# DerrickWang005/CRIS.pytorch

Hardware: AMD Instinct MI355X
Metric: train-step samples/sec, CRIS-R50 416x416 bs=64; loss parity vs ref (higher is better)
Workload: dtype bf16; 1 GPU; CRIS-R50 bf16 training step (fwd+BCE+bwd+Adam), 416x416, per-GPU bs=8, 17-token text, synthetic RefCOCO-shape batch resident in HBM (BASELINE.json configs[1]); global_batch=8, parallelism=dp1, launch=graph, graph_captured=True, syncbn_exchange=none, grad_exchange=none

## Files before the change

cris/pytorch_amd/csrc/build.py:

```python
import hashlib
import os
import subprocess
import sys

HERE = os.path.dirname(os.path.abspath(__file__))
SOURCES = ["api.hip", "gemm.hip", "gemm8.hip", "gemm_fp8.hip", "wgrad.hip", "norm.hip", "attention.hip", "elementwise.hip", "ema.hip", "lr.hip", "smallf32.hip", "evalpost.hip", "inputpipe.hip", "p2p.hip", "comm.hip", "jpeg.hip", "png.hip"]
LIB = os.path.join(HERE, "libcris_hip.so")
STAMP = os.path.join(HERE, ".build_stamp")
FLAGS = ["--offload-arch=gfx950", "-O3", "-std=c++17", "-fPIC", "-Wno-unused-result", "-fno-slp-vectorize", "-fno-vectorize"]
FLAGS += os.environ.get("CRIS_EXTRA_HIPCC_FLAGS", "").split()
OBJDUMP = "/opt/rocm/lib/llvm/bin/llvm-objdump"


def _digest():
    h = hashlib.sha256()
    for f in SOURCES + ["common.h", "gemm_common.h", "p2p_ll.h", "jpeg_core.h", os.path.join("..", "..", "..", "include", "cris_hip.h")]:
        with open(os.path.join(HERE, f), "rb") as fh:
            h.update(fh.read())
    h.update(" ".join(FLAGS).encode())
    return h.hexdigest()


def _current(dig):
    return os.path.exists(LIB) and os.path.exists(STAMP) and open(STAMP).read() == dig


def build(force=False, verbose=False):
    dig = _digest()
    if not force and _current(dig):
        return LIB
    import fcntl
    with open(os.path.join(HERE, ".build_lock"), "w") as lock:
        fcntl.flock(lock, fcntl.LOCK_EX)
        try:
            if not force and _current(dig):
                return LIB
            return _compile(dig, verbose)
        finally:
            fcntl.flock(lock, fcntl.LOCK_UN)


def packed_fp32_ops(lib=LIB):
    import re
    import shutil
    import tempfile
    if not os.path.exists(OBJDUMP):
        return None
    found = {}
    with tempfile.TemporaryDirectory() as td:
        so = os.path.join(td, "lib.so")
        shutil.copy(lib, so)
        subprocess.run([OBJDUMP, "--offloading", so], cwd=td, stdout=subprocess.DEVNULL, stderr=subprocess.DEVNULL)
        for f in sorted(os.listdir(td)):
            if "gfx950" not in f:
                continue
            asm = subprocess.run([OBJDUMP, "-d", os.path.join(td, f)], stdout=subprocess.PIPE, stderr=subprocess.DEVNULL).stdout.decode()
            name = "?"
            for line in asm.splitlines():
                m = re.match(r"^[0-9a-f]+ <(.*)>:", line)
# ... 49 lines not shown
```

cris/pytorch_amd/csrc/gemm.hip:

```cpp
#include "gemm_common.h"
#ifndef ST_64x64
#define ST_64x64 3
#endif
#ifndef ST_64x128
#define ST_64x128 3
#endif
#ifndef ST_128x64
#define ST_128x64 3
#endif
#ifndef ST_128x128
#define ST_128x128 2
#endif
#define SKINNY_MAX_M 144

#ifdef G4_PROBE
__device__ unsigned long long* g4_stamps;
#define G4_T(k) t_stamp[k] = __builtin_amdgcn_s_memtime()
#ifndef G4_ABL
#define G4_ABL 0
#endif
#else
#define G4_T(k)
#define G4_ABL 0
#endif


template <int BM, int BN, int WAVES_M, int WAVES_N, int STAGES, int EPI, int MT_ = 32, int KS = 1>
__device__ __forceinline__ void conv_gemm_tile(const cris_conv_gemm_params& p, int bid, unsigned char* smem) {
    constexpr int WTM = BM / WAVES_M;
    constexpr int WTN = BN / WAVES_N;
    constexpr int MT = MT_;
    using acc_t = typename std::conditional<MT == 32, f32x16, f32x4>::type;
    constexpr int FM = WTM / MT;
    constexpr int FN = WTN / MT;
    constexpr int NA = BM / 32;
    constexpr int NB = BN / 32;
    constexpr int A_BYTES = BM * 128;
    constexpr int STAGE_BYTES = (BM + BN) * 128;

#ifdef G4_PROBE
    unsigned long long t_stamp[6];
#endif
    G4_T(0);
    if (G4_ABL & 8) {
        if (p.M < 0) p.colsum[0] = 0.f;
        return;
    }
    const int t = threadIdx.x;
    const int lane = t & 63;
    const int wave = (t >> 6) & 3;
    const int grp = KS > 1 ? (t >> 8) : 0;
    unsigned char* const ring = smem + grp * (STAGES * STAGE_BYTES);
    const int wm = wave / WAVES_N;
    const int wn = wave % WAVES_N;

    const int tiles_n = (p.N + BN - 1) / BN;
    const int tiles_m = (p.M + BM - 1) / BM;
    int tile_m, tile_n;
    if ((long)p.N * p.K > (1L << 20)) {
        tile_n = cris_fast_div(bid, tiles_m, __builtin_amdgcn_rcpf((float)tiles_m));
        tile_m = bid - tile_n * tiles_m;
    } else {
        tile_m = cris_fast_div(bid, tiles_n, __builtin_amdgcn_rcpf((float)tiles_n));
        tile_n = bid - tile_m * tiles_n;
// ... 370 lines not shown
    }
    __syncthreads();
    if (wave == 0) {
        float* slab = p.ws + ((size_t)ks * gridDim.x + nb) * (FM * FN * 256);
#pragma unroll
        for (int i = 0; i < FM; ++i)
#pragma unroll
            for (int j = 0; j < FN; ++j) {
                f32x4 v = acc[i][j];
#pragma unroll
                for (int w = 0; w < SK2_WAVES - 1; ++w) {
                    const f32x4 o = *reinterpret_cast<const f32x4*>(&red[w][i * FN + j][lane][0]);
                    v[0] += o[0]; v[1] += o[1]; v[2] += o[2]; v[3] += o[3];
                }
                *reinterpret_cast<f32x4*>(slab + (i * FN + j) * 256 + lane * 4) = v;
            }
    }
}

template <int FM>
__global__ __launch_bounds__(256) void skinny_finish_kernel(const cris_conv_gemm_params p, int nslices, int nblocks) {
    const int lane = threadIdx.x & 63, wave = threadIdx.x >> 6;
    const int u = blockIdx.x * 4 + wave;
    const int nfc = nblocks * 2;
    if (u >= FM * nfc) return;
    const int i = u / nfc, c = u - i * nfc;
    const int nb = c >> 1, j = c & 1;
    f32x4 one[1][1];
    one[0][0] = (f32x4){0.f, 0.f, 0.f, 0.f};
    const float* src = p.ws + (size_t)nb * (FM * 2 * 256) + (i * 2 + j) * 256 + lane * 4;
    const size_t slab = (size_t)nblocks * (FM * 2 * 256);
    for (int k0 = 0; k0 < nslices; k0 += 4) {
        f32x4 o[4];
#pragma unroll
        for (int q = 0; q < 4; ++q) o[q] = *reinterpret_cast<const f32x4*>(src + (size_t)min(k0 + q, nslices - 1) * slab);
#pragma unroll
        for (int q = 0; q < 4; ++q)
            if (k0 + q < nslices) { one[0][0][0] += o[q][0]; one[0][0][1] += o[q][1]; one[0][0][2] += o[q][2]; one[0][0][3] += o[q][3]; }
    }
    gemm_epilogue<0, 16, 1, 1>(p, one, i * 16, c * 16, i, lane);
}

static int skinny_split_slices(const cris_conv_gemm_params& p) {
    static const int target = cris_env_int("CRIS_SKINNY_BLOCKS", 192);
    const int nblocks = cris_cdiv(p.N, 32);
    int ks = target / nblocks;
    const int kmax = p.K / 128;
    if (ks > kmax) ks = kmax;
    if (ks < 1) ks = 1;
    return ks;
}
static int skinny_kslice(const cris_conv_gemm_params& p, int slices) { return cris_cdiv(cris_cdiv(p.K, slices), 32) * 32; }

enum { V_SKINNY1 = 0, V_SKINNY9, V_SKINNY9S, V_128x64, V_64x64, V_64x128, V_128x128, V_8W_256x256, V_8W_256x128, V_8W_128x256, V_8W_128x128, V_64x64_K2, V_COUNT };

#define CRIS_TILE4_KERNS(K, BM, BN, WM, WN, ST) K<BM, BN, WM, WN, ST, 0>, K<BM, BN, WM, WN, ST, 1>, K<BM, BN, WM, WN, ST, 2>
#define CRIS_TILE4_ROW(NAME, BM, BN, WM, WN, ST)                                                                           \
    {NAME, BM, BN, 256, ST * (BM + BN) * 128, BM / WM, 8,                                                                  \
     {CRIS_TILE4_KERNS(conv_gemm_kernel, BM, BN, WM, WN, ST), conv_gemm_kernel<BM, BN, WM, WN, ST, 3>},                  \
     {CRIS_TILE4_KERNS(conv_gemm_group_kernel, BM, BN, WM, WN, ST)}}
static const cris_gemm_variant_desc* variant_table() {
    static const cris_gemm_variant_desc* const g8 = cris_gemm8_variants();
    static const cris_gemm_variant_desc tab[V_COUNT] = {
        {"skinny1", 16, 32, 64 * SK_WAVES, 0, 16, 8, {}, {}},
        {"skinny9", SKINNY_MAX_M, 32, 64 * SK_WAVES, 0, 16, 8, {}, {}},
        {"skinny9s", SKINNY_MAX_M, 32, 64 * SK2_WAVES, 0, 16, 8, {}, {}},
        CRIS_TILE4_ROW("128x64", 128, 64, 4, 1, ST_128x64),
        CRIS_TILE4_ROW("64x64", 64, 64, 2, 2, ST_64x64),
        CRIS_TILE4_ROW("64x128", 64, 128, 2, 2, ST_64x128),
        CRIS_TILE4_ROW("128x128", 128, 128, 2, 2, ST_128x128),
        g8[0], g8[1], g8[2], g8[3],
        {"64x64k2", 64, 64, 512, 2 * 2 * (64 + 64) * 128, 32, 8,
         {conv_gemm_kernel<64, 64, 2, 2, 2, 0, 32, 2>, conv_gemm_kernel<64, 64, 2, 2, 2, 1, 32, 2>, conv_gemm_kernel<64, 64, 2, 2, 2, 2, 32, 2>, nullptr},
         {}}};
    return tab;
}
static int variants_lds_ready() {
    static const int rc = [] {
        int rc = 0;
        for (int v = 0; v < V_COUNT; ++v) {
            const cris_gemm_variant_desc& r = variant_table()[v];
            for (int e = 0; e < 4; ++e) rc |= cris_set_lds((const void*)r.kern[e], r.lds_bytes);
            for (int e = 0; e < 3; ++e) rc |= cris_set_lds((const void*)r.group_kern[e], r.lds_bytes);
        }
        return rc;
    }();
    if (rc != 0) cris_set_error("gemm variants: hipFuncSetAttribute(MaxDynamicSharedMemorySize) failed (%d)", rc);
    return rc;
}

static int epilogue_kind(const cris_conv_gemm_params& p) {
    const bool plain = p.drop_thresh == 0u && !p.outT && p.out && !p.out_f32 && !(p.resid && p.resid_f32);
    if (plain && !p.bias && p.act == 0) return p.bnr_y ? 3 : 1;
    return !plain ? 0 : (p.act == 0 || p.act == 1 || p.act == 3) ? 2 : 0;
}

static bool variant_applicable(int v, const cris_conv_gemm_params& p) {
    if (v < 0 || v >= V_COUNT) return false;
    const cris_gemm_variant_desc& r = variant_table()[v];
    if (r.kern[0]) return p.C % r.c_mult == 0;
    const bool lin = p.KH == 1 && p.KW == 1 && p.stride == 1 && p.pad == 0 && p.OH == p.H && p.OW == p.W;
    return lin && p.M <= r.bm;
}

static int pick_variant(const cris_conv_gemm_params& p) {
    const bool lin = p.KH == 1 && p.KW == 1 && p.stride == 1 && p.pad == 0 && p.OH == p.H && p.OW == p.W;
    if (lin && p.M <= 16) return V_SKINNY1;
    static const int skinny_split = cris_env_int("CRIS_SKINNY_SPLIT", 1);
    if (lin && p.M <= SKINNY_MAX_M) {
        if (!skinny_split) return V_SKINNY9;
        return p.K >= 1024 ? V_SKINNY9S : V_64x64;
    }
    static const int g8 = cris_env_int("CRIS_GEMM8", 1);
    static const int g8_min = cris_env_int("CRIS_GEMM8_MIN_TILES", 150);
    static const int g8_min_k = cris_env_int("CRIS_GEMM8_MIN_K", 256);
    static const int g8_t128_lo = cris_env_int("CRIS_GEMM8_T128_LO", 100), g8_t128_hi = cris_env_int("CRIS_GEMM8_T128_HI", 216);
    if (g8 && epilogue_kind(p) != 0 && (p.C & 63) == 0 && p.N >= 128) {
        const long t128 = (long)cris_cdiv(p.M, 128) * cris_cdiv(p.N, 128);
        if (p.K >= 512 && t128 >= g8_t128_lo && t128 <= g8_t128_hi) return V_8W_128x128;
        if (p.N > 128 && p.K >= g8_min_k) {
            const long t256 = (long)cris_cdiv(p.M, 256) * cris_cdiv(p.N, 256);
            if (p.K >= 512 && t256 >= g8_min && !(t256 > 256 && t256 <= 400)) return V_8W_256x256;
            const long t128x256 = (long)cris_cdiv(p.M, 128) * cris_cdiv(p.N, 256);
            if (t128x256 >= g8_min && !(t128x256 > 256 && t128x256 <= 400) && (p.K >= 512 || t128x256 <= 256)) return V_8W_128x256;
        }
    }
    static const int narrow128 = cris_env_int("CRIS_GEMM_NARROW_128", 0);
    if (p.N <= 64) return narrow128 ? V_128x64 : V_64x64;
    static const int t128_min = cris_env_int("CRIS_GEMM_T128_MIN", 448);
    if (p.M <= 8192 || (long)cris_cdiv(p.M, 128) * cris_cdiv(p.N, 128) < t128_min) {
        static const int t64_max = cris_env_int("CRIS_GEMM_T64_MAX", 1024);
        const bool long_k = p.K >= 4096 && p.M >= 4096 && p.N >= 256;
        if (!long_k && (long)cris_cdiv(p.M, 64) * cris_cdiv(p.N, 128) < t64_max) {
            static const int ks2 = cris_env_int("CRIS_GEMM_KS2", 0), ks2_max = cris_env_int("CRIS_GEMM_KS2_MAX_BLOCKS", 512);
            static const int ks2_min_k = cris_env_int("CRIS_GEMM_KS2_MIN_K", 256);
            if (ks2 && p.K >= ks2_min_k && epilogue_kind(p) != 3 && (long)cris_cdiv(p.M, 64) * cris_cdiv(p.N, 64) <= ks2_max) return V_64x64_K2;
            return V_64x64;
        }
        return V_64x128;
    }
    return V_128x128;
}
static int variant_stat_rows(int v) { return variant_table()[v].stat_rows; }
static int resolve_variant(const cris_conv_gemm_params& p, int variant) {
    if (variant < 0) return pick_variant(p);
    return variant_applicable(variant, p) ? variant : -1;
}
extern "C" int cris_conv_gemm_stat_rows(const cris_conv_gemm_params* p) { return variant_stat_rows(pick_variant(*p)); }
extern "C" int cris_conv_gemm_variant_stat_rows(const cris_conv_gemm_params* p, int variant) {
    const int v = resolve_variant(*p, variant);
    return v < 0 ? -1 : variant_stat_rows(v);
}
extern "C" long cris_conv_gemm_ws_floats(const cris_conv_gemm_params* p, int variant) {
    const int v = resolve_variant(*p, variant);
    if (v != V_SKINNY9S) return 0;
    return (long)skinny_split_slices(*p) * cris_cdiv(p->N, 32) * (9 * 2 * 256);
}
extern "C" int cris_conv_gemm_plan(const cris_conv_gemm_params* p, int variant, int* epilogue) {
    if (epilogue) *epilogue = epilogue_kind(*p);
    return resolve_variant(*p, variant);
}
extern "C" int cris_conv_gemm_num_variants(void) { return V_COUNT; }
extern "C" const char* cris_conv_gemm_variant_name(int v) { return (v >= 0 && v < V_COUNT) ? variant_table()[v].name : "?"; }

extern "C" int cris_conv_gemm(const cris_conv_gemm_params* pp, void* stream) { return cris_conv_gemm_variant(pp, -1, stream); }

static int conv_gemm_check(const cris_conv_gemm_params& p);

extern "C" int cris_conv_gemm_group_launch(const cris_conv_gemm_group* gp, int variant, void* stream) {
    CRIS_CHECK_ARG(gp && gp->n > 0 && gp->n <= CRIS_GEMM_GROUP_MAX, "1 .. CRIS_GEMM_GROUP_MAX problems per launch");
    CRIS_CHECK_ARG(variant >= 0 && variant < V_COUNT && variant_table()[variant].group_kern[0],
                   "group launches run the 4-wave tiles or the 8-wave 128x128 tile");
    if (gp->n == 1) return cris_conv_gemm_variant(&gp->prob[0], variant, stream);
    const cris_gemm_variant_desc& r = variant_table()[variant];
    cris_conv_gemm_group g = *gp;
    const int epi = epilogue_kind(g.prob[0]);
    CRIS_CHECK_ARG(epi < 3, "BatchNorm-backward partials are not available in grouped launches");
    int start = 0;
    for (int i = 0; i < g.n; ++i) {
        const cris_conv_gemm_params& p = g.prob[i];
        if (conv_gemm_check(p) != 0) return -1;
        CRIS_CHECK_ARG(epilogue_kind(p) == epi, "the problems of a group must share the epilogue instantiation");
        CRIS_CHECK_ARG(variant_applicable(variant, p), "tile variant not applicable to a problem of the group");
        g.block_start[i] = start;
        start += cris_tile_blocks(r.bm, r.bn, p.M, p.N);
    }
    for (int i = g.n; i <= CRIS_GEMM_GROUP_MAX; ++i) g.block_start[i] = start;
    if (const int rc = variants_lds_ready()) return rc;
    return cris_launch_tile(r.group_kern[epi], start, r.threads, r.lds_bytes, (hipStream_t)stream, g);
}

static int conv_gemm_check(const cris_conv_gemm_params& p) {
    CRIS_CHECK_ARG(p.A && p.Wt, "null operand");
    CRIS_CHECK_ARG(p.M > 0 && p.N > 0 && p.K > 0, "empty problem");
    CRIS_CHECK_ARG((p.C & 7) == 0 && (p.lda & 7) == 0 && (p.a_coff & 7) == 0, "A channels/ld/offset must be multiples of 8");
    CRIS_CHECK_ARG((p.ldb & 7) == 0 && (p.K & 7) == 0 && p.ldb >= p.K, "W ld / K must be multiples of 8");
    CRIS_CHECK_ARG(p.K == p.KH * p.KW * p.C, "K != KH*KW*C");
    CRIS_CHECK_ARG(p.M == p.Bn * p.OH * p.OW, "M != Bn*OH*OW");
    CRIS_CHECK_ARG(p.M < (1 << 24) && (long)cris_cdiv(p.M, 64) * cris_cdiv(p.N, 64) < (1L << 22),
                   "more than 2^24 output rows / 2^22 tiles (the reciprocal index arithmetic of the prologue is exact below that)");
    CRIS_CHECK_ARG(p.out || p.outT || p.colsum, "no output");
    CRIS_CHECK_ARG(!p.bnr_y || (epilogue_kind(p) == 3 && p.colsum && p.colsq && p.bnr_mean && p.bnr_invstd && p.bnr_scale && p.bnr_shift &&
                                (p.bnr_ldy & 7) == 0 && (size_t)p.M * p.bnr_ldy * 2 < (1UL << 31)),
                   "BatchNorm-backward partials need the lean epilogue, both tables and the four coefficient vectors");
    CRIS_CHECK_ARG(p.stat_ld == 0 || p.stat_ld >= p.N, "stat_ld < N");
    CRIS_CHECK_ARG(!p.outT || ((p.T_E & 63) == 0 && p.T_L > 0 && (p.T_Lpad & 3) == 0 && p.T_Lpad >= p.T_L && p.M % p.T_L == 0),
                   "bad transposed-store geometry");
    CRIS_CHECK_ARG((uintptr_t)p.A % 16 == 0 && (uintptr_t)p.Wt % 16 == 0, "operands must be 16-byte aligned");
    CRIS_CHECK_ARG((long)p.M * p.N < (1L << 32) || p.drop_thresh == 0u, "dropout index overflow");
    CRIS_CHECK_ARG((size_t)p.Bn * p.H * p.W * p.lda * 2 < (1UL << 31) && ((size_t)p.N + 256) * p.ldb * 2 < (1UL << 31) &&
                       (!p.out || (size_t)p.M * p.ldc * 4 < (1UL << 31)) && (!p.resid || (size_t)p.M * p.ldr * 4 < (1UL << 31)),
                   "operand extent must stay below 2 GiB (32-bit buffer offsets)");
    return 0;
}

extern "C" int cris_conv_gemm_variant(const cris_conv_gemm_params* pp, int variant, void* stream) {
    const cris_conv_gemm_params& p = *pp;
    if (conv_gemm_check(p) != 0) return -1;
    hipStream_t s = (hipStream_t)stream;
    if (const int rc = variants_lds_ready()) return rc;
    int v = resolve_variant(p, variant);
    CRIS_CHECK_ARG(v >= 0, "tile variant not applicable to this problem");
    if (variant < 0 && v == V_SKINNY9S && !p.ws) v = V_SKINNY9;
    const cris_gemm_variant_desc& r = variant_table()[v];
    CRIS_CHECK_ARG(!p.bnr_y || r.kern[3],
                   "BatchNorm-backward partials: the 4-wave tiles and the 8-wave 128x128 tile only (cris_conv_gemm_plan tells which variant runs)");
    const int nblocks = cris_cdiv(p.N, r.bn);
    switch (v) {
        case V_SKINNY1: return cris_launch_tile(skinny_gemm_kernel<1>, nblocks, r.threads, 0, s, p);
        case V_SKINNY9: return cris_launch_tile(skinny_gemm_kernel<9>, nblocks, r.threads, 0, s, p);
        case V_SKINNY9S: {
            CRIS_CHECK_ARG(p.ws != nullptr, "the split-K skinny variant needs the workspace (cris_conv_gemm_ws_floats)");
            const int slices = skinny_split_slices(p);
            hipLaunchKernelGGL(skinny_split_kernel<9>, dim3(nblocks, slices), dim3(r.threads), 0, s, p, skinny_kslice(p, slices));
            hipLaunchKernelGGL(skinny_finish_kernel<9>, dim3(cris_cdiv(9 * nblocks * 2, 4)), dim3(256), 0, s, p, slices, nblocks);
            CRIS_LAUNCH_CHECK();
            return 0;
        }
        default: return cris_launch_tile(r.kern[epilogue_kind(p)], cris_tile_blocks(r.bm, r.bn, p.M, p.N), r.threads, r.lds_bytes, s, p);
    }
}

#define PACK_ELEMS 4096

__global__ __launch_bounds__(256) void pack_weights_kernel(const cris_pack_desc* __restrict__ tab, int n_desc) {
    int lo = 0, hi = n_desc - 1;
    const int bid = blockIdx.x;
    while (lo < hi) {
        const int mid = (lo + hi + 1) >> 1;
        if (tab[mid].block_start <= bid) lo = mid; else hi = mid - 1;
    }
    const cris_pack_desc d = tab[lo];
    const int lb = bid - d.block_start;
    const long nF = d.dstF ? (long)d.N * d.taps * d.Cpad : 0;
    const long blocksF = (nF + PACK_ELEMS - 1) / PACK_ELEMS;
    if (lb < blocksF) {
        const long base = (long)lb * PACK_ELEMS;
        for (int e = threadIdx.x; e < PACK_ELEMS; e += 256) {
            const long i = base + e;
            if (i >= nF) break;
            const int c = (int)(i % d.Cpad);
            const long r = i / d.Cpad;
            const int tap = (int)(r % d.taps);
            const int n = (int)(r / d.taps);
            float v = 0.f;
            if (c < d.Cin) v = d.src_transposed ? d.src[(size_t)c * d.N + n] : d.src[((size_t)n * d.Cin + c) * d.taps + tap];
            if (d.row_scale) v *= d.row_scale[n];
            const long ldF = d.ldF > 0 ? d.ldF : (long)d.taps * d.Cpad;
            d.dstF[(long)n * ldF + (long)tap * d.Cpad + c] = f2bf(v);
        }
    } else {
        __shared__ float tile[64][65];
        const int tn = (d.Npad + 63) / 64, tc = (d.Cin + 63) / 64;
        int r = lb - (int)blocksF;
        const int nt = r % tn; r /= tn;
        const int ct = r % tc;
// ... 40 lines not shown
```

cris/pytorch_amd/csrc/gemm_common.h:

```cpp
#pragma once
#include "common.h"
#include "../../../include/cris_hip.h"
#include <type_traits>

#define BK 64
#ifndef CRIS_FAST_EPILOGUE
#define CRIS_FAST_EPILOGUE 1
#endif
#ifndef CRIS_FAST_EPILOGUE_GEN
#define CRIS_FAST_EPILOGUE_GEN 1
#endif

__device__ __forceinline__ int cris_xcd_logical_block(int bid, int total) {
    const int q = total >> 3, r = total & 7;
    const int xcd = bid & 7, idx = bid >> 3;
    return (xcd < r ? xcd * (q + 1) : r * (q + 1) + (xcd - r) * q) + idx;
}

__device__ __forceinline__ int lds_off(int row, int chunk) {
    return row * 128 + (((chunk ^ (row >> 1)) & 7) << 4);
}

__device__ __forceinline__ bf16_t f2bf_hw(float x) { return __builtin_bit_cast(bf16_t, (__bf16)x); }

// ... 324 lines not shown
                    b0 += gg;
                    b1 += gg * ((yv[r] - b_mean) * b_inv);
                }
            }
            if (MT == 16) { b0 += __shfl_xor(b0, 16, 64); b1 += __shfl_xor(b1, 16, 64); }
            b0 += __shfl_xor(b0, 32, 64);
            b1 += __shfl_xor(b1, 32, 64);
            if (fg == 0 && cvalid && part_cnt > 0) {
                p.colsum[(size_t)part * sld + col] = b0;
                p.colsq[(size_t)part * sld + col] = b1;
            }
        } else if (p.colsum) {
            float s1 = 0.f;
#pragma unroll
            for (int ig = 0; ig < FM * NG; ++ig)
#pragma unroll
                for (int r = 0; r < 4; ++r) s1 += vals[ig][r];
            if (MT == 16) s1 += __shfl_xor(s1, 16, 64);
            s1 += __shfl_xor(s1, 32, 64);
            const float mu = part_cnt > 0 ? s1 / (float)part_cnt : 0.f;
            float q = 0.f;
#pragma unroll
            for (int ig = 0; ig < FM * NG; ++ig)
#pragma unroll
                for (int r = 0; r < 4; ++r) {
                    const int i = ig / NG, g = ig % NG;
                    const int m = row0 + i * MT + (MT == 16 ? fg * 4 : g * 8 + fg * 4) + r;
                    const float d = vals[ig][r] - mu;
                    q += (m < p.M) ? d * d : 0.f;
                }
            if (MT == 16) q += __shfl_xor(q, 16, 64);
            q += __shfl_xor(q, 32, 64);
            if (fg == 0 && cvalid && part_cnt > 0) {
                const int sld = p.stat_ld ? p.stat_ld : p.N;
                p.colsum[(size_t)part * sld + col] = s1;
                p.colsq[(size_t)part * sld + col] = q;
            }
        }
    }
}


typedef void (*cris_gemm_kern_t)(const cris_conv_gemm_params);
typedef void (*cris_gemm_group_kern_t)(const cris_conv_gemm_group);
struct cris_gemm_variant_desc {
    const char* name;
    int bm, bn;
    int threads, lds_bytes;
    int stat_rows;
    int c_mult;
    cris_gemm_kern_t kern[4];
    cris_gemm_group_kern_t group_kern[3];
};
const cris_gemm_variant_desc* cris_gemm8_variants();

static inline int cris_tile_blocks(int bm, int bn, int M, int N) { return cris_cdiv(M, bm) * cris_cdiv(N, bn); }
static inline int cris_set_lds(const void* kern, int bytes) {
    return kern ? (int)hipFuncSetAttribute(kern, hipFuncAttributeMaxDynamicSharedMemorySize, bytes) : 0;
}
template <typename KERN, typename ARG>
static int cris_launch_tile(KERN kern, int blocks, int threads, int lds_bytes, hipStream_t s, const ARG& arg) {
    hipLaunchKernelGGL(kern, dim3(blocks), dim3(threads), lds_bytes, s, arg);
    CRIS_LAUNCH_CHECK();
    return 0;
}
```

cris/pytorch_amd/hip.py:

```python
import contextlib
import ctypes as C
import os

import torch

_HERE = os.path.dirname(os.path.abspath(__file__))
LIB_PATH = os.path.join(_HERE, "csrc", "libcris_hip.so")
if os.environ.get("CRIS_LIB_VARIANT"):
    LIB_PATH = os.path.join(_HERE, "csrc", "variants", "libcris_hip_%s.so" % os.environ["CRIS_LIB_VARIANT"])

P, I, L, F, U = C.c_void_p, C.c_int, C.c_long, C.c_float, C.c_uint32


class ConvGemmParams(C.Structure):
    _fields_ = [("A", P), ("Wt", P), ("bias", P), ("resid", P), ("out", P), ("outT", P), ("colsum", P), ("colsq", P),
                ("T_sec_stride", L),
                ("lda", I), ("a_coff", I),
                ("Bn", I), ("H", I), ("W", I), ("C", I),
                ("OH", I), ("OW", I), ("KH", I), ("KW", I), ("stride", I), ("pad", I),
                ("ldb", I),
                ("M", I), ("N", I), ("K", I),
                ("act", I),
                ("ldr", I), ("r_coff", I), ("resid_f32", I),
                ("ldc", I), ("c_coff", I), ("out_f32", I),
# ... 193 lines not shown

class JpegImage(C.Structure):
    _fields_ = [("coef", P), ("planes", P), ("rgb", P), ("info", JpegInfo)]


class P2PParams(C.Structure):
    _fields_ = [("data", P), ("boxes", P), ("gen_dev", P), ("err", P),
                ("n", I), ("rank", I), ("world", I),
                ("slot", I), ("slots", I),
                ("max_floats", I),
                ("gen_host", I),
                ("spin_limit", I)]


class P2PLink(C.Structure):
    _fields_ = [("boxes", P), ("err", P), ("gen_dev", P),
                ("gen_host", I), ("rank", I), ("world", I),
                ("slot", I), ("slots", I), ("max_floats", I), ("spin_limit", I)]


class P2PArenaParams(C.Structure):
    _fields_ = [("arenas", P), ("lo", C.c_long), ("n", C.c_long), ("link", P2PLink), ("blocks", I)]


STRUCTS = {
    "cris_conv_gemm_params": ConvGemmParams, "cris_conv_gemm_group": ConvGemmGroup, "cris_wgrad_params": WgradParams, "cris_wgrad_group": WgradGroup, "cris_pack_desc": PackDesc,
    "cris_conv_gemm_fp8_params": ConvGemmFp8Params, "cris_pack_fp8_desc": PackFp8Desc,
    "cris_bn_apply_params": BnApplyParams, "cris_bn_bwd_params": BnBwdParams, "cris_ln_fwd_params": LnFwdParams,
    "cris_ln_bwd_params": LnBwdParams, "cris_sum_entry": SumEntry, "cris_sum_group": SumGroup, "cris_attn_params": AttnParams, "cris_adam_desc": AdamDesc, "cris_ema_desc": EmaDesc, "cris_p2p_params": P2PParams, "cris_p2p_link": P2PLink, "cris_p2p_arena_params": P2PArenaParams, "cris_zero_ranges": ZeroRanges,
    "cris_sample_desc": SampleDesc, "cris_eval_desc": EvalDesc, "cris_jpeg_info": JpegInfo, "cris_jpeg_image": JpegImage,
}

_SIGS = {
    "cris_last_error": (C.c_char_p, []),
    "cris_abi_version": (I, []),
    "cris_sizeof": (I, [C.c_char_p]),
    "cris_echo_conv_gemm": (L, [P]),
    "cris_conv_gemm": (I, [P, P]),
    "cris_conv_wgrad": (I, [P, P]),
    "cris_conv_wgrad_group": (I, [P, P]),
    "cris_conv_wgrad_tile": (I, [P]),
    "cris_wgrad_reduce": (I, [P, P]),
    "cris_wgrad_reduce_group": (I, [P, P]),
    "cris_wgrad_ws_floats": (L, [I, I, I, I]),
    "cris_pack_weights": (I, [P, I, I, P]),
    "cris_pack_blocks": (I, [P]),
    "cris_pack_block_elems": (I, []),
    "cris_conv_gemm_stat_rows": (I, [P]),
    "cris_conv_gemm_variant": (I, [P, I, P]),
    "cris_conv_gemm_variant_stat_rows": (I, [P, I]),
    "cris_conv_gemm_ws_floats": (L, [P, I]),
    "cris_conv_gemm_num_variants": (I, []),
    "cris_conv_gemm_plan": (I, [P, I, P]),
    "cris_conv_gemm_group_launch": (I, [P, I, P]),
    "cris_conv_gemm_variant_name": (C.c_char_p, [I]),
    "cris_conv_gemm_fp8": (I, [P, I, P]),
    "cris_conv_gemm_fp8_plan": (I, [P, I]),
    "cris_conv_gemm_fp8_num_variants": (I, []),
    "cris_conv_gemm_fp8_variant_name": (C.c_char_p, [I]),
    "cris_pack_weights_fp8": (I, [P, I, I, P]),
    "cris_avgpool2_fwd_fp8": (I, [P, I, I, I, I, I, I, P, I, I, P, I, I, I, P]),
    "cris_absmax_bf16": (I, [P, I, I, L, I, P, P, P]),
    "cris_absmax_ws_floats": (I, []),
    "cris_bn_partials_rows": (I, [I]),
    "cris_bn_finalize": (I, [P, P, I, I, F, F, P, P, P, P, F, F, I, P, P, P, P, P, P, P]),
    "cris_bn_sync_pack": (I, [P, P, P, F, I, P]),
    "cris_bn_sync_unpack": (I, [P, P, F, I, P]),
    "cris_colstats_bf16": (I, [P, I, I, I, I, I, P, P, P]),
    "cris_bn_eval_coeffs": (I, [P, P, P, P, F, I, P, P, P]),
    "cris_bn_apply": (I, [P, P]),
    "cris_bn_bwd_reduce": (I, [P, P]),
    "cris_bn_bwd_apply": (I, [P, P]),
    "cris_bn_bwd_ws_floats": (L, [P]),
    "cris_ln_bwd_parts": (I, [I]),
    "cris_sum_tables": (I, [P, P]),
    "cris_ln_fwd": (I, [P, P]),
    "cris_ln_bwd": (I, [P, P]),
    "cris_attn_fwd": (I, [P, P]),
    "cris_attn_bwd_dq": (I, [P, P]),
    "cris_attn_bwd_dkv": (I, [P, P]),
    "cris_stem_im2col": (I, [P, I, I, I, P, P]),
    "cris_avgpool2_fwd": (I, [P, I, I, I, I, I, I, P, I, I, P]),
    "cris_avgpool2_bwd": (I, [P, I, I, I, I, I, I, P, I, I, I, P]),
    "cris_upsample2_fwd": (I, [P, I, I, I, I, I, I, P, I, I, P]),
    "cris_upsample2_bwd": (I, [P, I, I, I, I, I, I, P, I, I, I, P]),
    "cris_fill_coords": (I, [P, I, I, I, I, I, I, P]),
    "cris_gather_samples_bf16": (I, [P, I, I, P, I, I, I, P, I, I, P]),
    "cris_add_bf16": (I, [P, I, I, P, I, I, P, I, I, I, I, P]),
    "cris_add_rowtable": (I, [P, I, P, I, P, I, I, I, P]),
    "cris_cast_f32_bf16": (I, [P, P, L, P]),
    "cris_cast_bf16_f32": (I, [P, P, L, I, P]),
    "cris_cast_f32_bf16_drop": (I, [P, P, L, F, U, U, U, P, P]),
    "cris_step_advance": (I, [P, P, P, P]),
    "cris_step_advance_micro": (I, [P, P, P, I, I, P]),
    "cris_axpy_f32": (I, [P, P, F, L, P]),
    "cris_grad_accumulate": (I, [P, P, L, I, P]),
    "cris_quickgelu_fwd": (I, [P, P, L, P]),
    "cris_quickgelu_bwd": (I, [P, P, P, L, P]),
    "cris_embed_fwd": (I, [P, P, P, I, I, I, P, P]),
    "cris_embed_bwd": (I, [P, P, I, I, I, P, P, P, P]),
    "cris_eot_gather": (I, [P, P, I, I, I, P, P, P]),
    "cris_eot_scatter_add": (I, [P, P, I, I, I, P, P]),
    "cris_eot_gather_ln_f32": (I, [P, P, P, P, P, P, I, I, I, P, P, P]),
    "cris_eot_scatter_add_f32": (I, [P, P, I, I, I, P, P]),
    "cris_linear_f32_small": (I, [P, I, P, I, I, P, I, I, I, P, I, I, P]),
    "cris_outer_sum_f32_small": (I, [P, I, P, I, I, I, I, P, I, P, P]),
# ... 159 lines not shown
```

cris/pytorch_amd/ops.py:

```python
from __future__ import annotations

import ctypes as C
import math
import os
from dataclasses import dataclass
from typing import Optional

import torch

from . import hip
from .hip import ptr

BF16 = torch.bfloat16


def _stream():
    return torch.cuda.current_stream().cuda_stream


def pad8(n: int) -> int:
    return (n + 7) // 8 * 8


def pad32(n: int) -> int:
# ... 55 lines not shown
    def __init__(self):
        self.items = []

    @classmethod
    def groupable(cls):
        if cls.GROUPABLE is None:
            names = gemm_variants()
            cls.GROUPABLE = {names.index(n) for n in ("128x64", "64x64", "64x128", "128x128", "8w128x128")}
        return cls.GROUPABLE

    def add(self, p, variant, keep, flops, nbytes, tag):
        epi = C.c_int(0)
        v = hip.load().cris_conv_gemm_plan(C.byref(p), variant, C.byref(epi))
        if v < 0:
            raise ValueError("GEMM tile variant %r cannot run this problem" % (variant,))
        self.items.append((p, v, epi.value, keep, flops, nbytes, tag))

    def __len__(self):
        return len(self.items)

    def flush(self):
        items, self.items = self.items, []
        if not items:
            return
        groups = {}
        for it in items:
            key = (it[1], it[2]) if (self.enabled and it[1] in self.groupable()) else ("solo", id(it))
            groups.setdefault(key, []).append(it)
        for key, its in groups.items():
            if key[0] == "solo":
                _launch_gemm(its[0][0], its[0][1], its[0][4], its[0][5], its[0][6])
                continue
            its.sort(key=lambda it: -it[0].K)
            for i in range(0, len(its), hip.GEMM_GROUP_MAX):
                chunk = its[i:i + hip.GEMM_GROUP_MAX]
                if len(chunk) == 1:
                    _launch_gemm(chunk[0][0], chunk[0][1], chunk[0][4], chunk[0][5], chunk[0][6])
                    continue
                grp = hip.ConvGemmGroup()
                grp.n = len(chunk)
                for j, it in enumerate(chunk):
                    grp.prob[j] = it[0]
                if KERNEL_TIMER is not None:
                    KERNEL_TIMER.launch("conv_gemm", sum(it[4] for it in chunk), sum(it[5] for it in chunk), "cris_conv_gemm_group_launch",
                                        C.byref(grp), key[0], tag="group of %d: %s" % (len(chunk), " + ".join(it[6] for it in chunk)), tile=True)
                else:
                    hip.call("cris_conv_gemm_group_launch", C.byref(grp), key[0], _stream())


def _launch_gemm(p, variant, flops, nbytes, tag):
    if KERNEL_TIMER is not None:
        v = hip.load().cris_conv_gemm_plan(C.byref(p), variant, None)
        KERNEL_TIMER.launch("skinny_gemm" if (p.M <= 144 and p.KH == 1) else "conv_gemm", flops, nbytes, "cris_conv_gemm_variant",
                            C.byref(p), variant, tag=tag, tile=gemm_variants()[v] not in ("skinny1", "skinny9", "skinny9s"))
        return
    hip.call("cris_conv_gemm_variant", C.byref(p), variant, _stream())


def conv_gemm(A, Wt, g: Geom, N: int, *, lda=None, a_coff=0, ldb=None, bias=None, act=0, resid=None, ldr=None, r_coff=0,
              out=None, ldc=None, c_coff=0, outT=None, T_L=0, T_Lpad=0, T_E=0, T_sec_stride=0, stats=False,
              drop: Drop = NO_DROP, variant: int = -1, queue: Optional[GemmQueue] = None, bnr: Optional[dict] = None):
    p = hip.ConvGemmParams()
    p.A, p.Wt, p.bias = ptr(A), ptr(Wt), ptr(bias)
    p.lda = lda if lda is not None else A.shape[-1]
    p.a_coff = a_coff
    p.Bn, p.H, p.W, p.C = g.Bn, g.H, g.W, g.C
    p.OH, p.OW, p.KH, p.KW, p.stride, p.pad = g.OH, g.OW, g.KH, g.KW, g.stride, g.pad
    p.ldb = ldb if ldb is not None else Wt.shape[-1]
    p.M, p.N, p.K = g.M, N, g.K
    p.act = act
    if resid is not None:
        p.resid = ptr(resid)
        p.ldr = ldr if ldr is not None else resid.shape[-1]
        p.r_coff = r_coff
        p.resid_f32 = 1 if resid.dtype == torch.float32 else 0
    if out is not None:
        p.out = ptr(out)
        p.ldc = ldc if ldc is not None else out.shape[-1]
        p.c_coff = c_coff
        p.out_f32 = 1 if out.dtype == torch.float32 else 0
    if outT is not None:
        p.outT = ptr(outT)
        p.T_L, p.T_Lpad, p.T_E, p.T_sec_stride = T_L, T_Lpad, T_E, T_sec_stride
    p.drop_p, p.drop_thresh, p.drop_seed, p.drop_stream = drop.p, drop.thresh, drop.seed & 0xFFFFFFFF, drop.stream
    p.drop_seed_dev = ptr(drop.dev)
    st = None
    if isinstance(variant, str):
        variant = gemm_variants().index(variant)
    rows = hip.load().cris_conv_gemm_variant_stat_rows(C.byref(p), variant)
    if rows < 0:
        raise ValueError("GEMM tile variant %r cannot run this problem" % (variant,))
    parts = None
    if bnr is not None:
        assert not stats
        epi = C.c_int(0)
        v = hip.load().cris_conv_gemm_plan(C.byref(p), variant, C.byref(epi))
        nparts = (g.M + rows - 1) // rows
        if gemm_variants()[v] not in ("128x64", "64x64", "64x128", "128x128", "8w128x128") or epi.value != 1 or nparts > BNR_MAX_PARTS:
            bnr = None
        else:
            parts = BnrParts(torch.empty(nparts, 2 * N, dtype=torch.float32, device=A.device), nparts)
            p.colsum, p.colsq, p.stat_ld = ptr(parts.t), parts.t.data_ptr() + 4 * N, 2 * N
            p.bnr_y, p.bnr_ldy, p.bnr_coff = ptr(bnr["y"]), bnr["ldy"], bnr["coff"]
            p.bnr_mean, p.bnr_invstd, p.bnr_scale, p.bnr_shift = ptr(bnr["mean"]), ptr(bnr["invstd"]), ptr(bnr["scale"]), ptr(bnr["shift"])
    if stats:
        st = Stats((g.M + rows - 1) // rows, N, rows, A.device)
        p.colsum, p.colsq = ptr(st[0]), ptr(st[1])
    nws = hip.load().cris_conv_gemm_ws_floats(C.byref(p), variant)
    ws = torch.empty(nws, dtype=torch.float32, device=A.device) if nws else None
    p.ws = ptr(ws)
    flops, nbytes, tag = 2.0 * g.M * N * g.K, 2.0 * (g.M * g.C + N * g.K + g.M * N), "M%d N%d K%d k%d" % (g.M, N, g.K, g.KH)
    if queue is not None:
        assert bnr is None and parts is None, "a queued launch cannot feed a BatchNorm backward that runs before the flush"
        queue.add(p, variant, (A, Wt, bias, resid, out, outT, drop.dev, ws, st.t if st is not None else None), flops, nbytes, tag)
        return st
    _launch_gemm(p, variant, flops, nbytes, tag)
    return parts if bnr is not None else st


BNR_MAX_PARTS = int(os.environ.get("CRIS_BNR_MAX_PARTS", "512"))
BNR_FUSE = os.environ.get("CRIS_BNR_FUSE", "1") == "1"


class BnrParts:
    __slots__ = ("t", "nparts")

    def __init__(self, t, nparts):
        self.t, self.nparts = t, nparts


def gemm_variants():
    lib = hip.load()
    return [lib.cris_conv_gemm_variant_name(i).decode() for i in range(lib.cris_conv_gemm_num_variants())]


class KernelTimer:

    def __init__(self):
        self.records = []
        self.tile_flags = []

    def launch(self, name, flops, nbytes, fn, *args, tag="", tile=False):
        s = torch.cuda.current_stream()
        e0, e1 = torch.cuda.Event(enable_timing=True), torch.cuda.Event(enable_timing=True)
        e0.record(s)
        hip.call(fn, *args, s.cuda_stream)
        e1.record(s)
        self.records.append((name, flops, nbytes, e0, e1, tag))
        self.tile_flags.append(bool(tile))

    def tile_family(self):
        d = dict(launches=0, ms=0.0, flops=0.0, bytes=0.0)
        for (name, fl, nb, e0, e1, _), t in zip(self.records, self.tile_flags):
            if t:
                d["launches"] += 1
                d["ms"] += e0.elapsed_time(e1)
                d["flops"] += fl
                d["bytes"] += nb
        return d

    def by_shape(self):
        out = {}
        for name, fl, nb, e0, e1, tag in self.records:
            d = out.setdefault((name, tag), dict(launches=0, ms=0.0, flops=0.0, bytes=0.0))
            d["launches"] += 1
            d["ms"] += e0.elapsed_time(e1)
            d["flops"] += fl
            d["bytes"] += nb
        return out

    def summary(self):
        out = {}
        for name, fl, nb, e0, e1, _ in self.records:
            d = out.setdefault(name, dict(launches=0, ms=0.0, flops=0.0, bytes=0.0))
            d["launches"] += 1
            d["ms"] += e0.elapsed_time(e1)
            d["flops"] += fl
            d["bytes"] += nb
        return out


KERNEL_TIMER = None


_WGRAD_BLOCKS = int(os.environ.get("CRIS_WGRAD_BLOCKS", "512"))
_WGRAD_GROUP_M = int(os.environ.get("CRIS_WGRAD_GROUP_M", "8192"))
# ... 975 lines not shown
```

include/cris_hip.h:

```cpp
#ifndef CRIS_HIP_H
#define CRIS_HIP_H
#include <stddef.h>
#include <stdint.h>
#ifdef __cplusplus
extern "C" {
#endif

typedef uint16_t cris_bf16;

const char* cris_last_error(void);
#define CRIS_ABI_VERSION 8
int cris_abi_version(void);
int cris_sizeof(const char* struct_name);
long cris_echo_conv_gemm(const void* conv_gemm_params);

typedef struct {
    const cris_bf16* A;
    const cris_bf16* Wt;
    const float* bias;
    const void* resid;
    void* out;
    cris_bf16* outT;
    float* colsum;
    float* colsq;
    long T_sec_stride;
    int lda, a_coff;
    int Bn, H, W, C;
    int OH, OW, KH, KW, stride, pad;
    int ldb;
    int M, N, K;
    int act;
    int ldr, r_coff, resid_f32;
    int ldc, c_coff, out_f32;
    int T_L, T_Lpad, T_E;
    float drop_p;
    uint32_t drop_thresh;
    uint32_t drop_seed, drop_stream;
    const uint32_t* drop_seed_dev;
    float* ws;
    const cris_bf16* bnr_y;
    const float* bnr_mean; const float* bnr_invstd; const float* bnr_scale; const float* bnr_shift;
    int bnr_ldy, bnr_coff;
    int stat_ld, pad_;
} cris_conv_gemm_params;
int cris_conv_gemm(const cris_conv_gemm_params* p, void* stream);
int cris_conv_gemm_stat_rows(const cris_conv_gemm_params* p);
int cris_conv_gemm_variant(const cris_conv_gemm_params* p, int variant, void* stream);
int cris_conv_gemm_variant_stat_rows(const cris_conv_gemm_params* p, int variant);
long cris_conv_gemm_ws_floats(const cris_conv_gemm_params* p, int variant);
int cris_conv_gemm_num_variants(void);
const char* cris_conv_gemm_variant_name(int variant);
int cris_conv_gemm_plan(const cris_conv_gemm_params* p, int variant, int* epilogue);

#define CRIS_GEMM_GROUP_MAX 12
typedef struct {
    int n;
    int block_start[CRIS_GEMM_GROUP_MAX + 1];
    cris_conv_gemm_params prob[CRIS_GEMM_GROUP_MAX];
} cris_conv_gemm_group;
int cris_conv_gemm_group_launch(const cris_conv_gemm_group* g, int variant, void* stream);

typedef struct {
    const cris_bf16* dY;
    const cris_bf16* X;
    float* dW;
    int ldy, y_coff, N_ld;
    int ldx, x_coff;
    int Bn, H, W, C;
    int OH, OW, KH, KW, stride, pad;
    int M, N, K;
    int ldw;
    int splits;
    int tile;
    int defer_reduce;
    float* dbias;
    float* ws;
} cris_wgrad_params;
int cris_conv_wgrad(const cris_wgrad_params* p, void* stream);
int cris_conv_wgrad_tile(const cris_wgrad_params* p);
long cris_wgrad_ws_floats(int M, int N, int ldw, int splits);
int cris_wgrad_reduce(const cris_wgrad_params* p, void* stream);

#define CRIS_WGRAD_GROUP_MAX 24
typedef struct {
    int n;
    int block_start[CRIS_WGRAD_GROUP_MAX + 1];
    cris_wgrad_params prob[CRIS_WGRAD_GROUP_MAX];
} cris_wgrad_group;
int cris_conv_wgrad_group(const cris_wgrad_group* g, void* stream);
int cris_wgrad_reduce_group(const cris_wgrad_group* g, void* stream);

typedef struct {
    const float* src;
    cris_bf16* dstF;
    cris_bf16* dstD;
    const float* row_scale;
    int N, Cin, taps, Cpad, Npad, src_transposed;
    int block_start;
    int ldF;
    int ldD;
    int pad_;
} cris_pack_desc;
int cris_pack_weights(const cris_pack_desc* dev_table, int n_desc, int total_blocks, void* stream);
int cris_pack_blocks(const cris_pack_desc* host_desc);
int cris_pack_block_elems(void);
// ... 393 lines not shown
```

Before: 673.4 samples/s.

## Add direct 3x3 conv kernel with LDS row ring for small-channel layers

After: 674.8 samples/s, median of 4. Within noise of the previous version (+0.2%).

```diff
diff --git a/cris/pytorch_amd/csrc/build.py b/cris/pytorch_amd/csrc/build.py
--- a/cris/pytorch_amd/csrc/build.py
+++ b/cris/pytorch_amd/csrc/build.py
@@ -4,7 +4,7 @@
 import sys
 
 HERE = os.path.dirname(os.path.abspath(__file__))
-SOURCES = ["api.hip", "gemm.hip", "gemm8.hip", "gemm_fp8.hip", "wgrad.hip", "norm.hip", "attention.hip", "elementwise.hip", "ema.hip", "lr.hip", "smallf32.hip", "evalpost.hip", "inputpipe.hip", "p2p.hip", "comm.hip", "jpeg.hip", "png.hip"]
+SOURCES = ["api.hip", "gemm.hip", "gemm8.hip", "conv3x3_direct.hip", "gemm_fp8.hip", "wgrad.hip", "norm.hip", "attention.hip", "elementwise.hip", "ema.hip", "lr.hip", "smallf32.hip", "evalpost.hip", "inputpipe.hip", "p2p.hip", "comm.hip", "jpeg.hip", "png.hip"]
 LIB = os.path.join(HERE, "libcris_hip.so")
 STAMP = os.path.join(HERE, ".build_stamp")
 FLAGS = ["--offload-arch=gfx950", "-O3", "-std=c++17", "-fPIC", "-Wno-unused-result", "-fno-slp-vectorize", "-fno-vectorize"]
diff --git a/cris/pytorch_amd/csrc/conv3x3_direct.hip b/cris/pytorch_amd/csrc/conv3x3_direct.hip
--- /dev/null
+++ b/cris/pytorch_amd/csrc/conv3x3_direct.hip
@@ -0,0 +1,153 @@
+#include "gemm_common.h"
+
+#define D3_STEP 128
+#define D3_ZERO_BYTES 1024
+#define D3_LDS_MAX (160 * 1024)
+
+struct d3_geom {
+    int slot_bytes, nslots, lds_bytes, steps_per_block, blocks;
+};
+
+template <int C>
+__device__ __forceinline__ int d3_swz(int x) { return C == 32 ? (x >> 2) & 3 : (x >> 1) & 7; }
+
+template <int C, int NH>
+__global__ __launch_bounds__(256, 2) void conv3x3_direct_kernel(const cris_conv_gemm_params p, int slot_bytes, int nslots, int steps_per_block) {
+    extern __shared__ __attribute__((aligned(16))) unsigned char smem[];
+    constexpr int FM = NH;
+    constexpr int CH = C / 8;
+    constexpr int KSL = C / 16;
+    constexpr int PIXB = C * 2;
+    const int t = threadIdx.x, lane = t & 63, wave = t >> 6;
+    const int wn = wave % NH, wm = wave / NH;
+    const int fr = lane & 31, fh = lane >> 5;
+    const int W = p.W, H = p.H;
+    const int rows_total = p.Bn * H;
+    const int nsteps = (p.M + D3_STEP - 1) / D3_STEP;
+    const int s0 = blockIdx.x * steps_per_block, s1 = min(nsteps, s0 + steps_per_block);
+    const unsigned zero_base = (unsigned)(nslots * slot_bytes);
+
+    for (int i = t * 16; i < D3_ZERO_BYTES; i += 256 * 16) *reinterpret_cast<uint4*>(smem + zero_base + i) = make_uint4(0u, 0u, 0u, 0u);
+
+    auto step_lo = [&](int s) { return max(0, (s * D3_STEP) / W - 1); };
+    auto step_hi = [&](int s) { return min(rows_total - 1, (min(p.M, (s + 1) * D3_STEP) - 1) / W + 1); };
+    const __amdgpu_buffer_rsrc_t rsA = __builtin_amdgcn_make_buffer_rsrc(
+        const_cast<bf16_t*>(p.A), 0, (int)((size_t)p.Bn * p.H * p.W * p.lda * 2), CRIS_BUF_FLAGS);
+    auto issue_row = [&](int G) {
+        unsigned char* slot = smem + (G % nslots) * slot_bytes;
+        const unsigned pix0 = (unsigned)G * (unsigned)W;
+        for (int ch = wave; ch * 1024 < slot_bytes; ch += 4) {
+            const int u = ch * 64 + lane;
+            const int x = u / CH, q = (u % CH) ^ d3_swz<C>(x);
+            const bool ok = x >= 1 && x <= W;
+            const unsigned off = ((pix0 + (unsigned)(x - 1)) * (unsigned)p.lda + (unsigned)(p.a_coff + q * 8)) * 2u;
+            __builtin_amdgcn_raw_ptr_buffer_load_lds(rsA, (lds_void_t*)(slot + ch * 1024), 16, ok ? off : CRIS_OOB, 0, 0, 0);
+        }
+    };
+    int loaded = step_hi(min(s0 + 1, s1 - 1));
+    for (int G = step_lo(s0); G <= loaded; ++G) issue_row(G);
+
+    bf16x8 bw[9][KSL];
+    {
+        const bf16_t* wrow = p.Wt + (size_t)(wn * 32 + fr) * p.ldb + fh * 8;
+#pragma unroll
+        for (int tap = 0; tap < 9; ++tap)
+#pragma unroll
+            for (int ks = 0; ks < KSL; ++ks) bw[tap][ks] = *reinterpret_cast<const bf16x8*>(wrow + tap * C + ks * 16);
+    }
+    CRIS_VMCNT(0);
+    __syncthreads();
+
+    for (int s = s0; s < s1; ++s) {
+        f32x16 acc[FM][1][1];
+#pragma unroll
+        for (int i = 0; i < FM; ++i) {
+#pragma unroll
+            for (int r = 0; r < 16; ++r) acc[i][0][0][r] = 0.f;
+            const int m = (s * 4 + wm * FM + i) * 32 + fr;
+            unsigned rb[3] = {zero_base, zero_base, zero_base}, rmask[3] = {0u, 0u, 0u};
+            int ow = 0;
+            if (m < p.M) {
+                const int G = m / W;
+                const int oh = G % H;
+                ow = m - G * W;
+                rb[1] = (unsigned)((G % nslots) * slot_bytes);
+                rmask[1] = ~0u;
+                if (oh > 0) { rb[0] = (unsigned)(((G - 1) % nslots) * slot_bytes); rmask[0] = ~0u; }
+                if (oh < H - 1) { rb[2] = (unsigned)(((G + 1) % nslots) * slot_bytes); rmask[2] = ~0u; }
+            }
+            unsigned xo[3], xs[3];
+#pragma unroll
+            for (int dx = 0; dx < 3; ++dx) {
+                xo[dx] = (unsigned)(ow + dx) * PIXB;
+                xs[dx] = (unsigned)d3_swz<C>(ow + dx) << 4;
+            }
+#pragma unroll
+            for (int tap = 0; tap < 9; ++tap) {
+                const int dy = tap / 3, dx = tap % 3;
+#pragma unroll
+                for (int ks = 0; ks < KSL; ++ks) {
+                    const unsigned a = rb[dy] + ((xo[dx] + ((unsigned)((ks * 2 + fh) << 4) ^ xs[dx])) & rmask[dy]);
+                    const bf16x8 af = *reinterpret_cast<const bf16x8*>(smem + a);
+                    acc[i][0][0] = __builtin_amdgcn_mfma_f32_32x32x16_bf16(af, bw[tap][ks], acc[i][0][0], 0, 0, 0);
+                }
+            }
+        }
+        CRIS_VMCNT(0);
+        __syncthreads();
+        if (s + 2 < s1) {
+            const int h = step_hi(s + 2);
+            for (int G = loaded + 1; G <= h; ++G) issue_row(G);
+            loaded = max(loaded, h);
+        }
+#pragma unroll
+        for (int i = 0; i < FM; ++i) {
+            const int tile = s * 4 + wm * FM + i;
+            if (tile * 32 < p.M) gemm_epilogue<1, 32, 1, 1>(p, acc[i], tile * 32, wn * 32, tile, lane);
+        }
+    }
+}
+
+static bool d3_plan(const cris_conv_gemm_params& p, d3_geom* g) {
+    if (!(p.KH == 3 && p.KW == 3 && p.stride == 1 && p.pad == 1 && p.OH == p.H && p.OW == p.W)) return false;
+    if (!((p.C == 32 || p.C == 64) && (p.N == 32 || p.N == 64)) || p.K != 9 * p.C) return false;
+    const long slot = ((long)(p.W + 2) * p.C * 2 + 1023) / 1024 * 1024;
+    const long nslots = (p.W + 2 * D3_STEP - 2) / p.W + 1 + 2;
+    const long lds = slot * nslots + D3_ZERO_BYTES;
+    if (lds > D3_LDS_MAX) return false;
+    if (g) {
+        g->slot_bytes = (int)slot;
+        g->nslots = (int)nslots;
+        g->lds_bytes = (int)lds;
+        static const int blocks_max = cris_env_int("CRIS_CONV3_DIRECT_BLOCKS", 512);
+        const int nsteps = cris_cdiv(p.M, D3_STEP);
+        const int cap = lds * 2 <= D3_LDS_MAX ? blocks_max : blocks_max / 2;
+        const int target = cap > 0 ? cap : 1;
+        g->steps_per_block = cris_cdiv(nsteps, target);
+        g->blocks = cris_cdiv(nsteps, g->steps_per_block);
+    }
+    return true;
+}
+
+bool cris_conv3x3_direct_applicable(const cris_conv_gemm_params& p) { return d3_plan(p, nullptr); }
+
+typedef void (*d3_kern_t)(const cris_conv_gemm_params, int, int, int);
+int cris_conv3x3_direct_launch(const cris_conv_gemm_params& p, hipStream_t s) {
+    static const d3_kern_t kerns[2][2] = {{conv3x3_direct_kernel<32, 1>, conv3x3_direct_kernel<32, 2>},
+                                          {conv3x3_direct_kernel<64, 1>, conv3x3_direct_kernel<64, 2>}};
+    static const int lds_rc = [] {
+        int rc = 0;
+        for (int c = 0; c < 2; ++c)
+            for (int n = 0; n < 2; ++n) rc |= cris_set_lds((const void*)kerns[c][n], D3_LDS_MAX);
+        return rc;
+    }();
+    if (lds_rc != 0) {
+        cris_set_error("conv3x3 direct: hipFuncSetAttribute(MaxDynamicSharedMemorySize) failed (%d)", lds_rc);
+        return lds_rc;
+    }
+    d3_geom g;
+    CRIS_CHECK_ARG(d3_plan(p, &g), "the direct 3x3 kernel cannot run this problem");
+    hipLaunchKernelGGL(kerns[p.C == 64][p.N == 64], dim3(g.blocks), dim3(256), g.lds_bytes, s, p, g.slot_bytes, g.nslots, g.steps_per_block);
+    CRIS_LAUNCH_CHECK();
+    return 0;
+}
diff --git a/cris/pytorch_amd/csrc/gemm.hip b/cris/pytorch_amd/csrc/gemm.hip
--- a/cris/pytorch_amd/csrc/gemm.hip
+++ b/cris/pytorch_amd/csrc/gemm.hip
@@ -10,6 +10,9 @@
 #endif
 #ifndef ST_128x128
 #define ST_128x128 2
+#endif
+#ifndef D3_MIN_M
+#define D3_MIN_M 131072
 #endif
 #define SKINNY_MAX_M 144
 
@@ -486,7 +489,8 @@
 }
 static int skinny_kslice(const cris_conv_gemm_params& p, int slices) { return cris_cdiv(cris_cdiv(p.K, slices), 32) * 32; }
 
-enum { V_SKINNY1 = 0, V_SKINNY9, V_SKINNY9S, V_128x64, V_64x64, V_64x128, V_128x128, V_8W_256x256, V_8W_256x128, V_8W_128x256, V_8W_128x128, V_64x64_K2, V_COUNT };
+enum { V_SKINNY1 = 0, V_SKINNY9, V_SKINNY9S, V_128x64, V_64x64, V_64x128, V_128x128, V_8W_256x256, V_8W_256x128, V_8W_128x256, V_8W_128x128, V_64x64_K2, V_COUNT,
+       V_DIRECT3 = V_COUNT };
 
 #define CRIS_TILE4_KERNS(K, BM, BN, WM, WN, ST) K<BM, BN, WM, WN, ST, 0>, K<BM, BN, WM, WN, ST, 1>, K<BM, BN, WM, WN, ST, 2>
 #define CRIS_TILE4_ROW(NAME, BM, BN, WM, WN, ST)                                                                           \
@@ -575,11 +579,18 @@
     }
     return V_128x128;
 }
-static int variant_stat_rows(int v) { return variant_table()[v].stat_rows; }
+static bool direct3_applicable(const cris_conv_gemm_params& p) { return epilogue_kind(p) == 1 && cris_conv3x3_direct_applicable(p); }
+static bool direct3_auto(const cris_conv_gemm_params& p) {
+    static const int on = cris_env_int("CRIS_CONV3_DIRECT", 1);
+    return on && p.M >= D3_MIN_M && direct3_applicable(p) && pick_variant(p) == V_64x64;
+}
+static int variant_stat_rows(int v) { return v == V_DIRECT3 ? 32 : variant_table()[v].stat_rows; }
 static int resolve_variant(const cris_conv_gemm_params& p, int variant) {
     if (variant < 0) return pick_variant(p);
+    if (variant == V_DIRECT3) return direct3_applicable(p) ? V_DIRECT3 : -1;
     return variant_applicable(variant, p) ? variant : -1;
 }
+extern "C" int cris_conv_gemm_direct(const cris_conv_gemm_params* p) { return direct3_auto(*p) ? 1 : 0; }
 extern "C" int cris_conv_gemm_stat_rows(const cris_conv_gemm_params* p) { return variant_stat_rows(pick_variant(*p)); }
 extern "C" int cris_conv_gemm_variant_stat_rows(const cris_conv_gemm_params* p, int variant) {
     const int v = resolve_variant(*p, variant);
@@ -595,7 +606,9 @@
     return resolve_variant(*p, variant);
 }
 extern "C" int cris_conv_gemm_num_variants(void) { return V_COUNT; }
-extern "C" const char* cris_conv_gemm_variant_name(int v) { return (v >= 0 && v < V_COUNT) ? variant_table()[v].name : "?"; }
+extern "C" const char* cris_conv_gemm_variant_name(int v) {
+    return v == V_DIRECT3 ? "3x3direct" : (v >= 0 && v < V_COUNT) ? variant_table()[v].name : "?";
+}
 
 extern "C" int cris_conv_gemm(const cris_conv_gemm_params* pp, void* stream) { return cris_conv_gemm_variant(pp, -1, stream); }
 
@@ -656,6 +669,7 @@
     int v = resolve_variant(p, variant);
     CRIS_CHECK_ARG(v >= 0, "tile variant not applicable to this problem");
     if (variant < 0 && v == V_SKINNY9S && !p.ws) v = V_SKINNY9;
+    if (v == V_DIRECT3 || (variant < 0 && direct3_auto(p))) return cris_conv3x3_direct_launch(p, s);
     const cris_gemm_variant_desc& r = variant_table()[v];
     CRIS_CHECK_ARG(!p.bnr_y || r.kern[3],
                    "BatchNorm-backward partials: the 4-wave tiles and the 8-wave 128x128 tile only (cris_conv_gemm_plan tells which variant runs)");
diff --git a/cris/pytorch_amd/csrc/gemm_common.h b/cris/pytorch_amd/csrc/gemm_common.h
--- a/cris/pytorch_amd/csrc/gemm_common.h
+++ b/cris/pytorch_amd/csrc/gemm_common.h
@@ -400,6 +400,8 @@
     cris_gemm_kern_t kern[4];
     cris_gemm_group_kern_t group_kern[3];
 };
+bool cris_conv3x3_direct_applicable(const cris_conv_gemm_params& p);
+int cris_conv3x3_direct_launch(const cris_conv_gemm_params& p, hipStream_t s);
 const cris_gemm_variant_desc* cris_gemm8_variants();
 
 static inline int cris_tile_blocks(int bm, int bn, int M, int N) { return cris_cdiv(M, bm) * cris_cdiv(N, bn); }
diff --git a/cris/pytorch_amd/hip.py b/cris/pytorch_amd/hip.py
--- a/cris/pytorch_amd/hip.py
+++ b/cris/pytorch_amd/hip.py
@@ -269,6 +269,7 @@
     "cris_conv_gemm_ws_floats": (L, [P, I]),
     "cris_conv_gemm_num_variants": (I, []),
     "cris_conv_gemm_plan": (I, [P, I, P]),
+    "cris_conv_gemm_direct": (I, [P]),
     "cris_conv_gemm_group_launch": (I, [P, I, P]),
     "cris_conv_gemm_variant_name": (C.c_char_p, [I]),
     "cris_conv_gemm_fp8": (I, [P, I, P]),
diff --git a/cris/pytorch_amd/ops.py b/cris/pytorch_amd/ops.py
--- a/cris/pytorch_amd/ops.py
+++ b/cris/pytorch_amd/ops.py
@@ -131,7 +131,7 @@
     if KERNEL_TIMER is not None:
         v = hip.load().cris_conv_gemm_plan(C.byref(p), variant, None)
         KERNEL_TIMER.launch("skinny_gemm" if (p.M <= 144 and p.KH == 1) else "conv_gemm", flops, nbytes, "cris_conv_gemm_variant",
-                            C.byref(p), variant, tag=tag, tile=gemm_variants()[v] not in ("skinny1", "skinny9", "skinny9s"))
+                            C.byref(p), variant, tag=tag, tile=gemm_variant_name(v) not in ("skinny1", "skinny9", "skinny9s"))
         return
     hip.call("cris_conv_gemm_variant", C.byref(p), variant, _stream())
 
@@ -165,7 +165,7 @@
     p.drop_seed_dev = ptr(drop.dev)
     st = None
     if isinstance(variant, str):
-        variant = gemm_variants().index(variant)
+        variant = gemm_variant_index(variant)
     rows = hip.load().cris_conv_gemm_variant_stat_rows(C.byref(p), variant)
     if rows < 0:
         raise ValueError("GEMM tile variant %r cannot run this problem" % (variant,))
@@ -175,7 +175,7 @@
         epi = C.c_int(0)
         v = hip.load().cris_conv_gemm_plan(C.byref(p), variant, C.byref(epi))
         nparts = (g.M + rows - 1) // rows
-        if gemm_variants()[v] not in ("128x64", "64x64", "64x128", "128x128", "8w128x128") or epi.value != 1 or nparts > BNR_MAX_PARTS:
+        if gemm_variant_name(v) not in ("128x64", "64x64", "64x128", "128x128", "8w128x128") or epi.value != 1 or nparts > BNR_MAX_PARTS:
             bnr = None
         else:
             parts = BnrParts(torch.empty(nparts, 2 * N, dtype=torch.float32, device=A.device), nparts)
@@ -211,6 +211,22 @@
 def gemm_variants():
     lib = hip.load()
     return [lib.cris_conv_gemm_variant_name(i).decode() for i in range(lib.cris_conv_gemm_num_variants())]
+
+
+def gemm_variant_name(v: int) -> str:
+    return hip.load().cris_conv_gemm_variant_name(v).decode()
+
+
+def gemm_variant_index(name: str) -> int:
+    names = gemm_variants()
+    if name in names:
+        return names.index(name)
+    v = len(names)
+    while gemm_variant_name(v) != "?":
+        if gemm_variant_name(v) == name:
+            return v
+        v += 1
+    raise ValueError("no GEMM variant named %r" % (name,))
 
 
 class KernelTimer:
diff --git a/include/cris_hip.h b/include/cris_hip.h
--- a/include/cris_hip.h
+++ b/include/cris_hip.h
@@ -51,6 +51,7 @@
 int cris_conv_gemm_num_variants(void);
 const char* cris_conv_gemm_variant_name(int variant);
 int cris_conv_gemm_plan(const cris_conv_gemm_params* p, int variant, int* epilogue);
+int cris_conv_gemm_direct(const cris_conv_gemm_params* p);
 
 #define CRIS_GEMM_GROUP_MAX 12
 typedef struct {
```
